# UCF-CRCV/TeD-SPAD

Measured on AMD Instinct MI355X. Metric: clips/sec (16x224^2 I3D features), higher is better.
Workload: dtype f16; 1 GPU; cfg2 dali_extraction path: largei3d extract_features, 225 clip times x 10 crops = 2250 clip-forwards of 3x16x224x224 per GPU per step, random-init weights; global_batch=375, parallelism=clip-sharded x1 + RCCL all-gather of (T,10,F) features

## Files before the change

ted_spad_amd/csrc/conv_flat.hip:

```cpp
#include "conv_common.h"

namespace tedspad {
namespace {

__device__ uint4 g_zero16f;

constexpr int FL_BM = 256;
constexpr int FL_WSTAGE = 64 * BK * 2;

struct FlatGeo {
    int W, H, R, NP, ntaps;
};

template <typename T>
__global__ __launch_bounds__(256) void conv_flat_kernel(const ConvKP p, const FlatGeo g) {
    constexpr int NT = 256, WS = 3;
    extern __shared__ __attribute__((aligned(16))) unsigned char dsm[];
    const int tid = threadIdx.x, lane = tid & 63;
    const int wave = __builtin_amdgcn_readfirstlane(tid >> 6);
    const int tile = xcd_remap(blockIdx.x, gridDim.x);
    const int q0 = tile * FL_BM;
    const int S = (g.NP + 1) * 8;
    const int Sr = (S + 63) / 64 * 64;
    const int halo_bytes = Sr * 16;
    unsigned char *wring = dsm + halo_bytes;
    const unsigned lds0 = (unsigned)(uintptr_t)(lptr_t)dsm;
    const uint16_t *zero = reinterpret_cast<const uint16_t *>(&g_zero16f);

    const int rsub = wave * 8 + (lane >> 3);
    const int kc = (lane & 7) ^ ((4 * (wave & 1) + (lane >> 4)) & 7);
    const uint16_t *wsrc = p.w + (size_t)rsub * p.Kpad + kc * 8;
    auto issue_w = [&](int kt, int slot) {
        const unsigned dst = lds0 + halo_bytes + slot * FL_WSTAGE + wave * 8 * (BK * 2);
        lds_dma16(wsrc + kt * BK, dst);
        lds_dma16(wsrc + (size_t)32 * p.Kpad + kt * BK, dst + 32 * (BK * 2));
    };
    issue_w(0, 0);
    const int NH = (Sr + NT - 1) / NT;
    for (int i = 0; i < NH; ++i) {
        if (i * NT + wave * 64 >= Sr) break;
        const int s = i * NT + tid;
        const int pos = s >> 3, cs = s & 7;
        const int q = q0 - g.R + pos;
        const bool ok = pos < g.NP && (unsigned)q < (unsigned)p.M;
        const uint16_t *src = ok ? p.x + (size_t)q * p.ldx + ((cs ^ ((pos >> 1) & 7)) << 3) : zero;
        lds_dma16(src, lds0 + (i * NT + wave * 64) * 16);
    }
    if (g.ntaps > 1) issue_w(1, 1);

    const int l31 = lane & 31, lh = lane >> 5;
    const int swz = (l31 >> 1) & 7;
    int pj[2];
    unsigned vmask[2];
#pragma unroll
    for (int b = 0; b < 2; ++b) {
        const int j = wave * 64 + b * 32 + l31;
        pj[b] = j;
        const int q = q0 + j;
        unsigned mk = 0;
        if (q < p.M) {
            const int r1 = q / g.W, w = q - r1 * g.W;
            const int h = r1 % g.H;
            for (int dh = 0; dh < p.kh; ++dh)
                for (int dw = 0; dw < p.kw; ++dw)
                    if ((unsigned)(h + dh - p.ph) < (unsigned)g.H && (unsigned)(w + dw - p.pw) < (unsigned)g.W) mk |= 1u << (dh * p.kw + dw);
        }
        vmask[b] = mk;
    }
    f32x16 acc[2][2];
#pragma unroll
    for (int a = 0; a < 2; ++a)
#pragma unroll
        for (int b = 0; b < 2; ++b)
#pragma unroll
            for (int r = 0; r < 16; ++r) acc[a][b][r] = 0.f;

    if (g.ntaps > 1) wait_vmcnt<2>(); else wait_vmcnt<0>();
    __builtin_amdgcn_s_barrier();
    asm volatile("" ::: "memory");
    int dh = 0, dw = 0;
    for (int kt = 0; kt < g.ntaps; ++kt) {
        const int delta = dh * g.W + dw;
        unsigned xoff[2], xswz[2];
#pragma unroll
        for (int b = 0; b < 2; ++b) {
            const int pos = ((vmask[b] >> kt) & 1u) ? pj[b] + delta : g.NP;
            xoff[b] = (unsigned)pos * 128u;
            xswz[b] = (unsigned)(pos >> 1) & 7u;
        }
        const uint4 fa00 = *reinterpret_cast<const uint4 *>(dsm + xoff[0] + (((unsigned)lh ^ xswz[0]) << 4));
        const uint4 fa01 = *reinterpret_cast<const uint4 *>(dsm + xoff[1] + (((unsigned)lh ^ xswz[1]) << 4));
        if (kt + 1 < g.ntaps) wait_vmcnt<2>(); else wait_vmcnt<0>();
        __builtin_amdgcn_s_barrier();
        asm volatile("" ::: "memory");
        if (kt + 2 < g.ntaps) issue_w(kt + 2, (kt + 2) % WS);
        const uint16_t *Wt = reinterpret_cast<const uint16_t *>(wring + (kt % WS) * FL_WSTAGE) + l31 * BK;
        {
            const unsigned c = (unsigned)lh;
            const uint4 fw0 = *reinterpret_cast<const uint4 *>(Wt + ((c ^ swz) << 3)), fw1 = *reinterpret_cast<const uint4 *>(Wt + 32 * BK + ((c ^ swz) << 3));
            acc[0][0] = T::mfma(fw0, fa00, acc[0][0]);
            acc[0][1] = T::mfma(fw0, fa01, acc[0][1]);
            acc[1][0] = T::mfma(fw1, fa00, acc[1][0]);
            acc[1][1] = T::mfma(fw1, fa01, acc[1][1]);
        }
#pragma unroll
        for (int ks = 1; ks < 4; ++ks) {
            const unsigned c = (unsigned)((ks << 1) | lh);
            uint4 fa[2], fw[2];
#pragma unroll
            for (int b = 0; b < 2; ++b) fa[b] = *reinterpret_cast<const uint4 *>(dsm + xoff[b] + ((c ^ xswz[b]) << 4));
#pragma unroll
            for (int a = 0; a < 2; ++a) fw[a] = *reinterpret_cast<const uint4 *>(Wt + a * 32 * BK + ((c ^ swz) << 3));
#pragma unroll
            for (int a = 0; a < 2; ++a)
#pragma unroll
                for (int b = 0; b < 2; ++b) acc[a][b] = T::mfma(fw[a], fa[b], acc[a][b]);
        }
        if (++dw == p.kw) { dw = 0; ++dh; }
    }
    __syncthreads();

    constexpr int STG_LD = 64 + 4;
    float *stg = reinterpret_cast<float *>(dsm);
#pragma unroll
    for (int a = 0; a < 2; ++a)
#pragma unroll
        for (int b = 0; b < 2; ++b) {
            const int ml = wave * 64 + b * 32 + l31;
#pragma unroll
            for (int qd = 0; qd < 4; ++qd) {
                f32x4 v = {acc[a][b][4 * qd], acc[a][b][4 * qd + 1], acc[a][b][4 * qd + 2], acc[a][b][4 * qd + 3]};
                *reinterpret_cast<f32x4 *>(stg + ml * STG_LD + a * 32 + 8 * qd + 4 * lh) = v;
            }
        }
    __syncthreads();
    const int cc = tid & 7, r0 = tid >> 3;
    const int nch = cc * 8;
    if (nch >= p.Cout) return;
    float sc[8], sf[8];
#pragma unroll
    for (int i = 0; i < 8; ++i) { sc[i] = p.scale[nch + i]; sf[i] = p.shift[nch + i]; }
#pragma unroll
    for (int it = 0; it < FL_BM / 32; ++it) {
        const int r = r0 + it * 32;
        const size_t m = (size_t)q0 + r;
        if (m >= (size_t)p.M) continue;
        const f32x4 v0 = *reinterpret_cast<const f32x4 *>(stg + r * STG_LD + nch);
        const f32x4 v1 = *reinterpret_cast<const f32x4 *>(stg + r * STG_LD + nch + 4);
        float v[8];
#pragma unroll
        for (int i = 0; i < 4; ++i) { v[i] = v0[i] * sc[i] + sf[i]; v[i + 4] = v1[i] * sc[i + 4] + sf[i + 4]; }
        if (p.res) {
            float rr[8];
            unpack8<T>(*reinterpret_cast<const uint4 *>(p.res + m * p.ldres + nch), rr);
#pragma unroll
            for (int i = 0; i < 8; ++i) v[i] += rr[i];
        }
        if (p.relu) {
#pragma unroll
            for (int i = 0; i < 8; ++i) v[i] = __builtin_fmaxf(v[i], 0.f);
        }
        *reinterpret_cast<uint4 *>(p.y + m * p.ldy + nch) = pack8_lim<T>(v, p.sat);
    }
}

template <typename T>
int32_t launch_flat_t(const ConvKP &p, hipStream_t s) {
    FlatGeo g;
    g.W = p.Wi; g.H = p.Hi; g.R = p.ph * p.Wi + p.pw; g.ntaps = p.kh * p.kw;
    g.NP = FL_BM + (p.kh - 1) * p.Wi + (p.kw - 1);
    const int S = (g.NP + 1) * 8;
    const int main_bytes = (S + 63) / 64 * 64 * 16 + 3 * FL_WSTAGE;
    const int stage_bytes = FL_BM * (64 + 4) * 4;
    const int lds = main_bytes > stage_bytes ? main_bytes : stage_bytes;
    if (lds > 160 * 1024) {
        set_error("tedspad_conv_fwd: flat-halo config: halo does not fit LDS (%d bytes)", lds);
        return TEDSPAD_EINVAL;
    }
    static thread_local int attr_set[2] = {0, 0};
    auto kfn = conv_flat_kernel<T>;
    if (!attr_set[T::kDtype]) {
        if (hipFuncSetAttribute((const void *)kfn, hipFuncAttributeMaxDynamicSharedMemorySize, 160 * 1024) != hipSuccess) {
            set_error("tedspad_conv_fwd: cannot raise the dynamic LDS limit");
            return TEDSPAD_ELAUNCH;
        }
        attr_set[T::kDtype] = 1;
    }
    const int tiles = (p.M + FL_BM - 1) / FL_BM;
    hipLaunchKernelGGL(kfn, dim3(tiles), dim3(256), lds, s, p, g);
    return check_launch("tedspad_conv_fwd(flat halo)");
}

struct TFlatGeo {
    int T, HW, tiles_s, nchunks, kt, pt;
};

template <typename T_>
__global__ __launch_bounds__(256) void conv_tflat_kernel(const ConvKP p, const TFlatGeo g) {
    constexpr int NT = 256;
    constexpr int NP = 256;
    constexpr int HALO = (NP + 8) * 128;
    extern __shared__ __attribute__((aligned(16))) unsigned char dsm[];
    const int tid = threadIdx.x, lane = tid & 63;
    const int wave = __builtin_amdgcn_readfirstlane(tid >> 6);
    const int tile = xcd_remap(blockIdx.x, gridDim.x);
    const int n = tile / g.tiles_s, s0 = (tile - n * g.tiles_s) * 64;
    unsigned char *wbuf = dsm + HALO;
    const unsigned lds0 = (unsigned)(uintptr_t)(lptr_t)dsm;
    const uint16_t *zero = reinterpret_cast<const uint16_t *>(&g_zero16f);

    const int rsub = wave * 8 + (lane >> 3);
    const int kc = (lane & 7) ^ ((4 * (wave & 1) + (lane >> 4)) & 7);
    const uint16_t *wsrc = p.w + (size_t)rsub * p.Kpad + kc * 8;
    int hsrc[9];
#pragma unroll
    for (int i = 0; i < 9; ++i) {
        const int s = i * NT + tid;
        const int pos = s >> 3, cs = s & 7;
        const int f = pos >> 6, px = pos & 63;
        hsrc[i] = -1;
        if (pos < NP && f < g.T && s0 + px < g.HW) hsrc[i] = (int)((((long)n * g.T + f) * g.HW + s0 + px) * p.ldx) + ((cs ^ ((pos >> 1) & 7)) << 3);
    }
    const int l31 = lane & 31, lh = lane >> 5;
    const int swz = (l31 >> 1) & 7;
    f32x16 acc[2][2];
#pragma unroll
    for (int a = 0; a < 2; ++a)
#pragma unroll
        for (int b = 0; b < 2; ++b)
#pragma unroll
            for (int r = 0; r < 16; ++r) acc[a][b][r] = 0.f;

    for (int ch = 0; ch < g.nchunks; ++ch) {
        if (ch) __builtin_amdgcn_s_barrier();
        asm volatile("" ::: "memory");
#pragma unroll
        for (int i = 0; i < 9; ++i) {
            if (i * NT + wave * 64 >= (NP + 8) * 8) break;
            lds_dma16(hsrc[i] >= 0 ? p.x + hsrc[i] + ch * 64 : zero, lds0 + (i * NT + wave * 64) * 16);
        }
        for (int dt = 0; dt < g.kt; ++dt) {
            const unsigned dst = lds0 + HALO + dt * FL_WSTAGE + wave * 8 * (BK * 2);
            const uint16_t *src = wsrc + dt * p.cin + ch * 64;
            lds_dma16(src, dst);
            lds_dma16(src + (size_t)32 * p.Kpad, dst + 32 * (BK * 2));
        }
        wait_vmcnt<0>();
        __builtin_amdgcn_s_barrier();
        asm volatile("" ::: "memory");
        for (int dt = 0; dt < g.kt; ++dt) {
            const int fin = wave + dt - g.pt;
            if (wave >= g.T || fin < 0 || fin >= g.T) continue;
            const uint16_t *Wt = reinterpret_cast<const uint16_t *>(wbuf + dt * FL_WSTAGE) + l31 * BK;
            unsigned xoff[2], xswz[2];
#pragma unroll
            for (int b = 0; b < 2; ++b) {
                const int pos = fin * 64 + b * 32 + l31;
                xoff[b] = (unsigned)pos * 128u;
                xswz[b] = (unsigned)(pos >> 1) & 7u;
            }
#pragma unroll
            for (int ks = 0; ks < 4; ++ks) {
                const unsigned c = (unsigned)((ks << 1) | lh);
                uint4 fa[2], fw[2];
#pragma unroll
                for (int b = 0; b < 2; ++b) fa[b] = *reinterpret_cast<const uint4 *>(dsm + xoff[b] + ((c ^ xswz[b]) << 4));
#pragma unroll
                for (int a = 0; a < 2; ++a) fw[a] = *reinterpret_cast<const uint4 *>(Wt + a * 32 * BK + ((c ^ swz) << 3));
#pragma unroll
                for (int a = 0; a < 2; ++a)
#pragma unroll
                    for (int b = 0; b < 2; ++b) acc[a][b] = T_::mfma(fw[a], fa[b], acc[a][b]);
            }
        }
    }
    __syncthreads();

    constexpr int STG_LD = 64 + 4;
    float *stg = reinterpret_cast<float *>(dsm);
#pragma unroll
    for (int a = 0; a < 2; ++a)
#pragma unroll
        for (int b = 0; b < 2; ++b) {
            const int ml = wave * 64 + b * 32 + l31;
#pragma unroll
            for (int qd = 0; qd < 4; ++qd) {
                f32x4 v = {acc[a][b][4 * qd], acc[a][b][4 * qd + 1], acc[a][b][4 * qd + 2], acc[a][b][4 * qd + 3]};
                *reinterpret_cast<f32x4 *>(stg + ml * STG_LD + a * 32 + 8 * qd + 4 * lh) = v;
            }
        }
    __syncthreads();
    const int cc = tid & 7, r0 = tid >> 3;
    const int nch = cc * 8;
    if (nch >= p.Cout) return;
    float sc[8], sf[8];
#pragma unroll
    for (int i = 0; i < 8; ++i) { sc[i] = p.scale[nch + i]; sf[i] = p.shift[nch + i]; }
#pragma unroll
    for (int it = 0; it < 8; ++it) {
        const int r = r0 + it * 32;
        const int f = r >> 6, px = r & 63;
        if (f >= g.T || s0 + px >= g.HW) continue;
        const size_t m = ((size_t)n * g.T + f) * g.HW + s0 + px;
        const f32x4 v0 = *reinterpret_cast<const f32x4 *>(stg + r * STG_LD + nch);
        const f32x4 v1 = *reinterpret_cast<const f32x4 *>(stg + r * STG_LD + nch + 4);
        float v[8];
#pragma unroll
        for (int i = 0; i < 4; ++i) { v[i] = v0[i] * sc[i] + sf[i]; v[i + 4] = v1[i] * sc[i + 4] + sf[i + 4]; }
        if (p.res) {
            float rr[8];
            unpack8<T_>(*reinterpret_cast<const uint4 *>(p.res + m * p.ldres + nch), rr);
#pragma unroll
            for (int i = 0; i < 8; ++i) v[i] += rr[i];
        }
        if (p.relu) {
#pragma unroll
            for (int i = 0; i < 8; ++i) v[i] = __builtin_fmaxf(v[i], 0.f);
        }
        *reinterpret_cast<uint4 *>(p.y + m * p.ldy + nch) = pack8_lim<T_>(v, p.sat);
    }
}

template <typename T_>
int32_t launch_tflat_t(const ConvKP &p, int N, int cin, hipStream_t s) {
    TFlatGeo g;
    g.T = p.Ti; g.HW = p.Hi * p.Wi; g.tiles_s = (g.HW + 63) / 64; g.nchunks = cin / 64; g.kt = p.kt; g.pt = p.pt;
    const int main_bytes = (256 + 8) * 128 + p.kt * FL_WSTAGE;
    const int stage_bytes = FL_BM * (64 + 4) * 4;
    const int lds = main_bytes > stage_bytes ? main_bytes : stage_bytes;
    static thread_local int attr_set[2] = {0, 0};
    auto kfn = conv_tflat_kernel<T_>;
    if (!attr_set[T_::kDtype]) {
        if (hipFuncSetAttribute((const void *)kfn, hipFuncAttributeMaxDynamicSharedMemorySize, 160 * 1024) != hipSuccess) {
            set_error("tedspad_conv_fwd: cannot raise the dynamic LDS limit");
            return TEDSPAD_ELAUNCH;
        }
        attr_set[T_::kDtype] = 1;
    }
    hipLaunchKernelGGL(kfn, dim3(N * g.tiles_s), dim3(256), lds, s, p, g);
    return check_launch("tedspad_conv_fwd(temporal flat halo)");
}

}

int32_t launch_conv_flat(int dtype, const ConvKP &p, int cin, hipStream_t s) {
    const bool same = p.To == p.Ti && p.Ho == p.Hi && p.Wo == p.Wi && p.pt == 0 && p.ph < p.kh && p.pw < p.kw;
    if (cin != 64 || p.kt != 1 || p.st != 1 || p.sh != 1 || p.sw != 1 || !same || p.kh * p.kw < 2 || p.kh * p.kw > 32 || p.Cout > 64 ||
        p.Kpad != p.kh * p.kw * 64 || p.mask || p.stats || p.ostrided || p.y32 || p.sigmoid || !p.y) {
        set_error("tedspad_conv_fwd: flat-halo config needs a stride-1 'same' 1 x kh x kw conv with cin = 64, cout <= 64 and the plain epilogue");
        return TEDSPAD_EINVAL;
    }
    return dtype == TEDSPAD_F16 ? launch_flat_t<F16>(p, s) : launch_flat_t<BF16>(p, s);
}

}

namespace tedspad {

int32_t launch_conv_tflat(int dtype, const ConvKP &p, int N, int cin, hipStream_t s) {
    const bool same = p.To == p.Ti && p.Ho == p.Hi && p.Wo == p.Wi && p.ph == 0 && p.pw == 0 && p.pt < p.kt;
    if (cin % 64 != 0 || p.kh != 1 || p.kw != 1 || p.kt < 2 || p.kt > 3 || p.st != 1 || p.sh != 1 || p.sw != 1 || !same || p.Ti > 4 || p.Cout > 64 ||
        p.Kpad != p.kt * cin || p.mask || p.stats || p.ostrided || p.y32 || p.sigmoid || !p.y) {
        set_error("tedspad_conv_fwd: temporal flat-halo config needs a stride-1 'same' kt x 1 x 1 conv (kt 2..3) with cin %% 64 == 0, cout <= 64, T <= 4");
        return TEDSPAD_EINVAL;
    }
    return dtype == TEDSPAD_F16 ? launch_tflat_t<F16>(p, N, cin, s) : launch_tflat_t<BF16>(p, N, cin, s);
}

}
```

Measured before the change: 24590 clips/s.

## Add persistent streaming temporal flat-halo conv kernel with multi-buffered LDS DMA

Adds a persistent-grid variant of the temporal kt x 1 x 1 conv. Each workgroup loads all weight chunks into LDS once, then walks tiles with an NB-deep ring of async LDS DMA halo buffers, so the next chunk's loads overlap the current chunk's MFMA work. The grid is sized to the CU count (overridable by env) instead of one block per tile. Residual add is fused into the epilogue and stores use inline-asm global stores. This removes per-tile weight reloads and launch/tail costs, but the vmcnt accounting and persistent scheduling add complexity and possible lower occupancy.

```diff
diff --git a/ted_spad_amd/csrc/conv_flat.hip b/ted_spad_amd/csrc/conv_flat.hip
--- a/ted_spad_amd/csrc/conv_flat.hip
+++ b/ted_spad_amd/csrc/conv_flat.hip
@@ -1,3 +1,5 @@
+#include <stdlib.h>
+
 #include "conv_common.h"
 
 namespace tedspad {
@@ -341,6 +343,241 @@
     return check_launch("tedspad_conv_fwd(temporal flat halo)");
 }
 
+typedef unsigned u32x4 __attribute__((ext_vector_type(4)));
+
+__device__ __forceinline__ void gstore16(void *dst, u32x4 v) {
+    asm volatile("global_store_dwordx4 %0, %1, off\n\ts_nop 1" ::"v"(dst), "v"(v) : "memory");
+}
+
+constexpr int TF_HB = 256 * 128;
+constexpr int TF_NBMAX = 4;
+
+template <int NB>
+__device__ __forceinline__ void tflat_wait_landed(int nep) {
+    if (nep == 0) wait_vmcnt<8 * (NB - 1)>();
+    else if (nep == 1) wait_vmcnt<8 * NB>();
+    else if (NB >= 2 && nep == 2) wait_vmcnt<8 * (NB + 1)>();
+    else if (NB >= 3 && nep == 3) wait_vmcnt<8 * (NB + 2)>();
+    else wait_vmcnt<8 * (NB + (NB >= 4 ? 3 : 0))>();
+}
+
+template <typename T_, int NB, bool RES>
+__global__ __launch_bounds__(256) void conv_tflat_stream_kernel(const ConvKP p, const TFlatGeo g, const int ntiles) {
+    extern __shared__ __attribute__((aligned(16))) unsigned char dsm[];
+    const int tid = threadIdx.x, lane = tid & 63;
+    const int wave = __builtin_amdgcn_readfirstlane(tid >> 6);
+    const int G = gridDim.x;
+    const int lid = xcd_remap(blockIdx.x, G);
+    const int wbytes = g.nchunks * g.kt * FL_WSTAGE;
+    const unsigned lds0 = (unsigned)(uintptr_t)(lptr_t)dsm;
+    const unsigned halo0 = lds0 + wbytes;
+    const uint16_t *zero = reinterpret_cast<const uint16_t *>(&g_zero16f);
+
+    {
+        const int rsub = wave * 8 + (lane >> 3);
+        const int kc = (lane & 7) ^ ((4 * (wave & 1) + (lane >> 4)) & 7);
+        const uint16_t *wsrc = p.w + (size_t)rsub * p.Kpad + kc * 8;
+        for (int ch = 0; ch < g.nchunks; ++ch)
+            for (int dt = 0; dt < g.kt; ++dt) {
+                const unsigned dst = lds0 + (ch * g.kt + dt) * FL_WSTAGE + wave * 8 * (BK * 2);
+                const uint16_t *src = wsrc + dt * p.cin + ch * 64;
+                lds_dma16(src, dst);
+                lds_dma16(src + (size_t)32 * p.Kpad, dst + 32 * (BK * 2));
+            }
+    }
+    const int hpx = tid >> 3;
+    const int hcs = ((tid & 7) ^ ((tid >> 4) & 7)) << 3;
+    int hoff[8];
+#pragma unroll
+    for (int i = 0; i < 8; ++i) hoff[i] = ((i >> 1) * g.HW + (i & 1) * 32 + hpx) * p.ldx + hcs;
+    int it_tile = lid, it_ch = 0, it_buf = 0;
+    const uint16_t *it_base = p.x;
+    unsigned it_ok = 0;
+    auto set_tile = [&](int tile) {
+        it_ok = 0;
+        if (tile < ntiles) {
+            const int n = tile / g.tiles_s, s0 = (tile - n * g.tiles_s) * 64;
+            it_base = p.x + ((size_t)n * g.T * g.HW + s0) * p.ldx;
+#pragma unroll
+            for (int i = 0; i < 8; ++i)
+                if ((i >> 1) < g.T && s0 + (i & 1) * 32 + hpx < g.HW) it_ok |= 1u << i;
+        }
+    };
+    auto issue_next = [&]() {
+#pragma unroll
+        for (int i = 0; i < 8; ++i)
+            lds_dma16(((it_ok >> i) & 1u) ? it_base + hoff[i] + it_ch * 64 : zero, halo0 + it_buf * TF_HB + (i * 256 + wave * 64) * 16);
+        if (++it_ch == g.nchunks) { it_ch = 0; it_tile += G; set_tile(it_tile); }
+        if (++it_buf == NB) it_buf = 0;
+    };
+    set_tile(it_tile);
+#pragma unroll
+    for (int i = 0; i < NB; ++i) issue_next();
+
+    const int l31 = lane & 31, lh = lane >> 5;
+    const int swz = (l31 >> 1) & 7;
+    float sc[2][16], sf[2][16];
+#pragma unroll
+    for (int a = 0; a < 2; ++a)
+#pragma unroll
+        for (int q = 0; q < 4; ++q) {
+            const int c = a * 32 + 8 * q + 4 * lh;
+            f32x4 v0 = {0.f, 0.f, 0.f, 0.f}, v1 = {0.f, 0.f, 0.f, 0.f};
+            if (c < p.Cout) {
+                v0 = *reinterpret_cast<const f32x4 *>(p.scale + c);
+                v1 = *reinterpret_cast<const f32x4 *>(p.shift + c);
+            }
+#pragma unroll
+            for (int j = 0; j < 4; ++j) { sc[a][4 * q + j] = v0[j]; sf[a][4 * q + j] = v1[j]; }
+        }
+#pragma unroll
+    for (int a = 0; a < 2; ++a)
+#pragma unroll
+        for (int r = 0; r < 16; ++r) asm volatile("" : "+v"(sc[a][r]), "+v"(sf[a][r]));
+    f32x16 acc[2][2];
+#pragma unroll
+    for (int a = 0; a < 2; ++a)
+#pragma unroll
+        for (int b = 0; b < 2; ++b)
+#pragma unroll
+            for (int r = 0; r < 16; ++r) acc[a][b][r] = 0.f;
+
+    unsigned hist = 0;
+    int buf = 0;
+    for (int tile = lid; tile < ntiles; tile += G) {
+        for (int ch = 0; ch < g.nchunks; ++ch) {
+            tflat_wait_landed<NB>(__builtin_popcount(hist & ((1u << NB) - 1u)));
+            __builtin_amdgcn_s_barrier();
+            asm volatile("" ::: "memory");
+            const unsigned char *hb = dsm + wbytes + buf * TF_HB;
+            for (int dt = 0; dt < g.kt; ++dt) {
+                const int fin = wave + dt - g.pt;
+                if (wave >= g.T || fin < 0 || fin >= g.T) continue;
+                const uint16_t *Wt = reinterpret_cast<const uint16_t *>(dsm + (ch * g.kt + dt) * FL_WSTAGE) + l31 * BK;
+                const unsigned char *xb = hb + (unsigned)(fin * 64 + l31) * 128u;
+#pragma unroll
+                for (int ks = 0; ks < 4; ++ks) {
+                    const unsigned c = (unsigned)((ks << 1) | lh);
+                    uint4 fa[2], fw[2];
+#pragma unroll
+                    for (int b = 0; b < 2; ++b) fa[b] = *reinterpret_cast<const uint4 *>(xb + b * 32 * 128 + ((c ^ swz) << 4));
+#pragma unroll
+                    for (int a = 0; a < 2; ++a) fw[a] = *reinterpret_cast<const uint4 *>(Wt + a * 32 * BK + ((c ^ swz) << 3));
+#pragma unroll
+                    for (int a = 0; a < 2; ++a)
+#pragma unroll
+                        for (int b = 0; b < 2; ++b) acc[a][b] = T_::mfma(fw[a], fa[b], acc[a][b]);
+                }
+            }
+            asm volatile("" ::: "memory");
+            __builtin_amdgcn_s_barrier();
+            asm volatile("" ::: "memory");
+            issue_next();
+            if (++buf == NB) buf = 0;
+            hist <<= 1;
+        }
+        const int n = tile / g.tiles_s, s0 = (tile - n * g.tiles_s) * 64;
+        if (wave < g.T) {
+#pragma unroll
+            for (int b = 0; b < 2; ++b) {
+                const int px = s0 + b * 32 + l31;
+                const bool inb = px < g.HW;
+                const size_t m = ((size_t)n * g.T + wave) * g.HW + (inb ? px : 0);
+#pragma unroll
+                for (int a = 0; a < 2; ++a) {
+                    unsigned r[4][2];
+                    if (RES) {
+#pragma unroll
+                        for (int qp = 0; qp < 2; ++qp) {
+                            const int c0 = a * 32 + qp * 16 + 8 * lh;
+                            uint4 rv = make_uint4(0, 0, 0, 0);
+                            if (inb && c0 < p.Cout) rv = load16_opaque(p.res + m * p.ldres + c0);
+                            const unsigned w4[4] = {rv.x, rv.y, rv.z, rv.w};
+#pragma unroll
+                            for (int h = 0; h < 2; ++h) {
+                                auto sw = __builtin_amdgcn_permlane32_swap(w4[h], w4[2 + h], false, false);
+                                r[2 * qp][h] = sw[0];
+                                r[2 * qp + 1][h] = sw[1];
+                            }
+                        }
+                    }
+                    unsigned d[4][2];
+#pragma unroll
+                    for (int q = 0; q < 4; ++q)
+#pragma unroll
+                        for (int h = 0; h < 2; ++h) {
+                            float v[2];
+#pragma unroll
+                            for (int e = 0; e < 2; ++e) {
+                                const int k = 4 * q + 2 * h + e;
+                                float t = acc[a][b][k] * sc[a][k] + sf[a][k];
+                                if (RES) t += T_::to_f32((uint16_t)(e ? r[q][h] >> 16 : r[q][h] & 0xffffu));
+                                if (p.relu) t = __builtin_fmaxf(t, 0.f);
+                                v[e] = t;
+                                acc[a][b][k] = 0.f;
+                            }
+                            d[q][h] = (unsigned)T_::from_f32_lim(v[0], p.sat) | ((unsigned)T_::from_f32_lim(v[1], p.sat) << 16);
+                        }
+#pragma unroll
+                    for (int q = 0; q < 4; q += 2)
+#pragma unroll
+                        for (int h = 0; h < 2; ++h) {
+                            auto sw = __builtin_amdgcn_permlane32_swap(d[q][h], d[q + 1][h], false, false);
+                            d[q][h] = sw[0];
+                            d[q + 1][h] = sw[1];
+                        }
+                    uint16_t *dst = p.y + m * p.ldy + a * 32 + 8 * lh;
+                    if (inb && a * 32 + 8 * lh < p.Cout) gstore16(dst, u32x4{d[0][0], d[0][1], d[1][0], d[1][1]});
+                    if (inb && a * 32 + 16 + 8 * lh < p.Cout) gstore16(dst + 16, u32x4{d[2][0], d[2][1], d[3][0], d[3][1]});
+                }
+            }
+            if (s0 + 64 <= g.HW && p.Cout == 64) hist |= 1u;
+        }
+    }
+    wait_vmcnt<0>();
+}
+
+int g_tflat_cus = 0;
+
+template <typename T_, int NB>
+int32_t launch_tflat_stream_nb(const ConvKP &p, const TFlatGeo &g, int N, int lds, hipStream_t s) {
+    if (!g_tflat_cus) {
+        int dev = 0, n = 0;
+        if (hipGetDevice(&dev) != hipSuccess || hipDeviceGetAttribute(&n, hipDeviceAttributeMultiprocessorCount, dev) != hipSuccess || n <= 0) n = 256;
+        g_tflat_cus = n;
+    }
+    const char *nwg_s = getenv("TEDSPAD_TFLAT_NWG");
+    const int nwg_env = nwg_s ? atoi(nwg_s) : 0;
+    const int ntiles = N * g.tiles_s;
+    int grid = nwg_env > 0 ? nwg_env : g_tflat_cus;
+    if (grid > ntiles) grid = ntiles;
+    static thread_local int attr_set[2][2] = {{0, 0}, {0, 0}};
+    const int res = p.res ? 1 : 0;
+    auto kfn = res ? conv_tflat_stream_kernel<T_, NB, true> : conv_tflat_stream_kernel<T_, NB, false>;
+    if (!attr_set[T_::kDtype][res]) {
+        if (hipFuncSetAttribute((const void *)kfn, hipFuncAttributeMaxDynamicSharedMemorySize, 160 * 1024) != hipSuccess) {
+            set_error("tedspad_conv_fwd: cannot raise the dynamic LDS limit");
+            return TEDSPAD_ELAUNCH;
+        }
+        attr_set[T_::kDtype][res] = 1;
+    }
+    hipLaunchKernelGGL(kfn, dim3(grid), dim3(256), lds, s, p, g, ntiles);
+    return check_launch("tedspad_conv_fwd(temporal flat halo, streaming)");
+}
+
+template <typename T_>
+int32_t launch_tflat_any(const ConvKP &p, int N, int cin, hipStream_t s) {
+    const char *sw = getenv("TEDSPAD_TFLAT_STREAM");
+    const int wbytes = (cin / 64) * p.kt * FL_WSTAGE;
+    int nb = (160 * 1024 - wbytes) / TF_HB;
+    if ((sw && atoi(sw) == 0) || nb < 2 || N <= 0) return launch_tflat_t<T_>(p, N, cin, s);
+    if (nb > TF_NBMAX) nb = TF_NBMAX;
+    TFlatGeo g;
+    g.T = p.Ti; g.HW = p.Hi * p.Wi; g.tiles_s = (g.HW + 63) / 64; g.nchunks = cin / 64; g.kt = p.kt; g.pt = p.pt;
+    const int lds = wbytes + nb * TF_HB;
+    return nb == 2 ? launch_tflat_stream_nb<T_, 2>(p, g, N, lds, s) : nb == 3 ? launch_tflat_stream_nb<T_, 3>(p, g, N, lds, s) : launch_tflat_stream_nb<T_, 4>(p, g, N, lds, s);
+}
+
 }
 
 int32_t launch_conv_flat(int dtype, const ConvKP &p, int cin, hipStream_t s) {
@@ -364,7 +601,7 @@
         set_error("tedspad_conv_fwd: temporal flat-halo config needs a stride-1 'same' kt x 1 x 1 conv (kt 2..3) with cin %% 64 == 0, cout <= 64, T <= 4");
         return TEDSPAD_EINVAL;
     }
-    return dtype == TEDSPAD_F16 ? launch_tflat_t<F16>(p, N, cin, s) : launch_tflat_t<BF16>(p, N, cin, s);
-}
-
-}
+    return dtype == TEDSPAD_F16 ? launch_tflat_any<F16>(p, N, cin, s) : launch_tflat_any<BF16>(p, N, cin, s);
+}
+
+}
```

New measurement: 24650 clips/s, median of 6. About the same (+0.2%).
